# acids-ircam/RAVE

Hardware: NVIDIA H100
Metric: audio-seconds/s (v2 train step fwd+bwd, 48 kHz) (higher is better)
Workload: dtype bf16

## Files before the change

include/rave_b200.h:

```cpp
#ifndef RAVE_B200_H
#define RAVE_B200_H

#include <stddef.h>
#include <stdint.h>

#ifdef __cplusplus
extern "C" {
#endif

#define RAVE_ACT_NONE 0
#define RAVE_ACT_LEAKY 1
#define RAVE_ACT_SNAKE 2

#define RAVE_PREC_FP32 0
#define RAVE_PREC_BF16 1
#define RAVE_PREC_TF32 2

int rave_b200_version(void);
const char *rave_b200_last_error(void);
unsigned long long rave_b200_launch_count(void);

int rave_pqmf_analysis_fwd(const float *x, const float *taps, float *y, int B, int T, int Lout,
                           int ntaps, int pad_l, int flip_sign, void *stream);
int rave_pqmf_synthesis_fwd(const float *x, const float *w, float *out, int B, int L, int K,
// ... 19 lines not shown
                          int Lq, int K, int stride, int dil, int pad_l, long os_a, long os_c,
                          int act_p, int act_q, float slope, const float *alpha, void *workspace,
                          void *stream);

int rave_weight_norm_fwd(const float *v, const float *g, float *w, float *norm_out, int C0, int R,
                         void *stream);
int rave_weight_norm_bwd(const float *dw, const float *v, const float *g, const float *norm,
                         float *dv, float *dg, int C0, int R, void *stream);

int rave_act_fwd(const float *x, float *y, int B, int C, int L, int act, float slope,
                 const float *alpha, void *stream);
int rave_act_bwd(const float *dy, const float *x, float *dx, float *dalpha, int B, int C, int L,
                 int act, float slope, const float *alpha, void *stream);
int rave_am_tanh_fwd(const float *x, float *y, int B, int C, int L, void *stream);
int rave_am_tanh_bwd(const float *dy, const float *x, float *dx, int B, int C, int L, void *stream);
int rave_reparam_fwd(const float *z, const float *eps, float *zs, float *kl_sum, int B, int C, int L, void *stream);

int rave_conv1d_tc_supported(int Cin, int Cout, int K, int stride, int dil);
int rave_dilated_unit_tc_supported(int C, int L);
int rave_dilated_unit_tc_fwd(const void *xa_bf16, const void *w3t_bf16, const void *w1t_bf16, void *a1_out,
                             float *out_f32, void *out_act, int B, int C, int L, int pitch, int dil, int pad_l,
                             float slope_in, float slope_mid, int act_out, float slope_out, void *stream);
int rave_conv1d_tc_plan(int B, int Cin, int Cout, int Lout, int K);
int rave_conv1d_tc_fwd(const void *xa_bf16, const void *wt_bf16, const float *bias, const float *res,
                       const void *res_bf16, const void *dact_src_bf16, const void *res_act_bf16, float res_slope,
                       float *out_f32, void *out_act_bf16,
                       int B, int Cin, int Lin, int in_pitch, int Cout, int Lout,
                       int K, int stride, int dil, int pad_l, int act, float slope, int out_rows,
                       int out_row_stride, int out_row_offset, const float *fm_d, int fm_bh, void *stream);
int rave_conv1d_tc_fwd_x3(const void *xa_bf16, const void *wt_bf16, const float *bias, const float *res,
                          const void *res_act, float res_slope, float *out_f32, void *out_act, int B, int Cin, int Lin,
                          int in_pitch, int Cout, int Lout, int K, int stride, int dil, int pad_l, int act, float slope,
                          int out_rows, int out_row_stride, int out_row_offset, int act_cs, void *stream);
int rave_conv1d_tc_wgrad_splits(int B, int Cm, int Lp, int Cn, int K);
int rave_time_stack_cl(const float *x, void *out_bf16, int B, int C, int T, int F, int Fp, int Cp, int kt, int pt,
                       void *stream);
int rave_time_stack_cl_bwd(const void *g_bf16, float *gx, int B, int C, int T, int F, int Fp, int Cp, int kt, int pt,
                           void *stream);
int rave_time_stack_nhwc(const float *x, void *out_bf16, int B, int C, int T, int F, long sb, long st, int Fp, int Cp, int kt,
                         int pt, void *stream);
int rave_time_stack_nhwc_bwd(const void *g_bf16, float *gx, int B, int C, int T, int F, int Fp, int Cp, int kt, int pt,
                             void *stream);
int rave_time_stack_nhwc_dil(const float *x, void *out_bf16, int B, int C, int T, int F, long sb, long st, int Fp, int Cp,
                             int kt, int pt, int dil, void *stream);
int rave_time_stack_nhwc_dil_bwd(const void *g_bf16, float *gx, int B, int C, int T, int F, int Fp, int Cp, int kt, int pt,
                                 int dil, void *stream);
// ... 109 lines not shown
```

rave_b200/_lib.py:

```python
import ctypes
import os
from ctypes import c_float, c_int, c_long, c_size_t, c_ulonglong, c_void_p, c_char_p

_HERE = os.path.dirname(os.path.abspath(__file__))
LIB_PATH = os.path.join(_HERE, "csrc", "librave_b200.so")

_P, _I, _F, _L = c_void_p, c_int, c_float, c_long

SIGNATURES = {
    "rave_b200_version": (c_int, []),
    "rave_b200_last_error": (c_char_p, []),
    "rave_b200_launch_count": (c_ulonglong, []),
    "rave_pqmf_analysis_fwd": (c_int, [_P, _P, _P, _I, _I, _I, _I, _I, _I, _P]),
    "rave_pqmf_synthesis_fwd": (c_int, [_P, _P, _P, _I, _I, _I, _I, _F, _I, _P]),
    "rave_pqmf_analysis_fast": (c_int, [_P, _P, _P, _P, _I, _I, _I, _I, _I, _P]),
    "rave_pqmf_synthesis_fast": (c_int, [_P, _P, _P, _P, _I, _I, _I, _F, _I, _P]),
    "rave_conv1d_gather_f32": (c_int, [_P, _P, _P, _P, _P, _I, _I, _I, _I, _I, _I, _I, _I, _I, _L, _L,
                                       _I, _F, _P, _I, _F, _P, _P, _P]),
    "rave_conv1d_scatter_f32": (c_int, [_P, _P, _P, _P, _P, _I, _I, _I, _I, _I, _I, _I, _I, _I, _L, _L,
                                        _I, _F, _P, _I, _F, _P, _P, _P]),
    "rave_conv1d_wgrad_workspace_bytes": (c_size_t, [_I, _I, _I, _I, _I]),
    "rave_conv1d_wgrad_f32": (c_int, [_P, _P, _P, _I, _I, _I, _I, _I, _I, _I, _I, _I, _L, _L, _I, _I,
                                      _F, _P, _P, _P]),
    "rave_weight_norm_fwd": (c_int, [_P, _P, _P, _P, _I, _I, _P]),
    "rave_weight_norm_bwd": (c_int, [_P, _P, _P, _P, _P, _P, _I, _I, _P]),
    "rave_act_fwd": (c_int, [_P, _P, _I, _I, _I, _I, _F, _P, _P]),
    "rave_act_bwd": (c_int, [_P, _P, _P, _P, _I, _I, _I, _I, _F, _P, _P]),
    "rave_am_tanh_fwd": (c_int, [_P, _P, _I, _I, _I, _P]),
    "rave_am_tanh_bwd": (c_int, [_P, _P, _P, _I, _I, _I, _P]),
    "rave_reparam_fwd": (c_int, [_P, _P, _P, _P, _I, _I, _I, _P]),
    "rave_conv1d_tc_supported": (c_int, [_I, _I, _I, _I, _I]),
    "rave_dilated_unit_tc_supported": (c_int, [_I, _I]),
    "rave_dilated_unit_tc_fwd": (c_int, [_P, _P, _P, _P, _P, _P, _I, _I, _I, _I, _I, _I, _F, _F, _I, _F, _P]),
    "rave_conv1d_tc_plan": (c_int, [_I, _I, _I, _I, _I]),
    "rave_conv1d_tc_fwd": (c_int, [_P, _P, _P, _P, _P, _P, _P, _F, _P, _P, _I, _I, _I, _I, _I, _I, _I, _I, _I, _I, _I,
                                   _F, _I, _I, _I, _P, _I, _P]),
    "rave_conv1d_tc_fwd_x3": (c_int, [_P, _P, _P, _P, _P, _F, _P, _P, _I, _I, _I, _I, _I, _I, _I, _I, _I, _I, _I, _F, _I,
                                      _I, _I, _I, _P]),
    "rave_weight_prep_tc_multi_x3": (c_int, [_I, _P, _P]),
    "rave_ncl_to_cl_x3": (c_int, [_P, _P, _I, _I, _I, _P]),
    "rave_conv1d_tc_wgrad": (c_int, [_P, _P, _P, _P, _I, _I, _I, _I, _I, _I, _I, _I, _I, _I, _I, _P]),
    "rave_tapmajor_to_weight_f32": (c_int, [_P, _P, _I, _I, _I, _I, _I, _P]),
    "rave_conv1d_tc_wgrad_splits": (c_int, [_I, _I, _I, _I, _I]),
    "rave_time_stack_cl": (c_int, [_P, _P, _I, _I, _I, _I, _I, _I, _I, _I, _P]),
    "rave_time_stack_cl_bwd": (c_int, [_P, _P, _I, _I, _I, _I, _I, _I, _I, _I, _P]),
    "rave_time_stack_nhwc": (c_int, [_P, _P, _I, _I, _I, _I, ctypes.c_long, ctypes.c_long, _I, _I, _I, _I, _P]),
    "rave_time_stack_nhwc_bwd": (c_int, [_P, _P, _I, _I, _I, _I, _I, _I, _I, _I, _P]),
    "rave_time_stack_nhwc_dil": (c_int, [_P, _P, _I, _I, _I, _I, ctypes.c_long, ctypes.c_long, _I, _I, _I, _I, _I, _P]),
    "rave_time_stack_nhwc_dil_bwd": (c_int, [_P, _P, _I, _I, _I, _I, _I, _I, _I, _I, _I, _P]),
    "rave_l1_stats_f32": (c_int, [_P, _P, _P, ctypes.c_long, _P]),
    "rave_leaky_fm_fwd": (c_int, [_P, _P, _P, ctypes.c_long, ctypes.c_float, _P]),
    "rave_leaky_fm_bwd": (c_int, [_P, _P, _P, _P, ctypes.c_long, ctypes.c_float, _P]),
    "rave_leaky_fm_stack_fwd": (c_int, [_P, _P, _P, _P, ctypes.c_long, _I, _I, _I, _I, ctypes.c_float, _P]),
    "rave_leaky_fm_stack_bwd": (c_int, [_P, _P, _P, _P, _P, ctypes.c_long, _I, _I, _I, _I, ctypes.c_float, _P]),
    "rave_leaky_fm_stack_dil_fwd": (c_int, [_P, _P, _P, _P, ctypes.c_long, _I, _I, _I, _I, _I, ctypes.c_float, _P]),
    "rave_leaky_fm_stack_dil_bwd": (c_int, [_P, _P, _P, _P, _P, ctypes.c_long, _I, _I, _I, _I, _I, ctypes.c_float, _P]),
    "rave_l1_grad_f32": (c_int, [_P, _P, _P, _P, _P, ctypes.c_long, _P]),
# ... 119 lines not shown
```

rave_b200/csrc/api.cu:

```cuda
#include <stdarg.h>

#include <atomic>

#include "common.cuh"

namespace rave {
static thread_local char g_err[512] = "";
static std::atomic<unsigned long long> g_launches{0};

void set_error(const char *fmt, ...) {
  va_list ap;
  va_start(ap, fmt);
  vsnprintf(g_err, sizeof(g_err), fmt, ap);
  va_end(ap);
}
void count_launch(int n) { g_launches.fetch_add((unsigned long long)n, std::memory_order_relaxed); }
}

extern "C" int rave_b200_version(void) { return 105; }
extern "C" const char *rave_b200_last_error(void) { return rave::g_err; }
extern "C" unsigned long long rave_b200_launch_count(void) {
  return rave::g_launches.load(std::memory_order_relaxed);
}
```

rave_b200/csrc/conv_tc.cu:

```cuda
#include <string.h>

#include "common.cuh"
#include "tc_common.cuh"

namespace rave {
namespace tc {

constexpr int BLOCK_M = 128;
constexpr int NUM_THREADS = 288;
constexpr int SMEM_MAX = 227 * 1024;

struct TcParams {
  int B, Cin, Lin, Cout, Lout, K, stride, dil, pad_l;
  int BL, BB;
  int n_lt, n_bg, n_nt;
  int num_kb;
  int act;
  float slope;
  const float *bias;
  const float *res;
  const __nv_bfloat16 *res_bf16;
  const __nv_bfloat16 *dact_src;
  const __nv_bfloat16 *res_act;
  float res_inv_slope;
  float *out_f32;
  __nv_bfloat16 *out_act;
  int out_rows;
  int out_row_stride;
  int out_row_offset;
  const float *fm_d;
  long fm_half;
  int fm_bh;
  int x3;
  int act_ld;
  int act_cs;
  int stages, nacc;
  int stg;
  int acc_off, stg_off, bar_off;
};

template <int BLOCK_N, int BLOCK_K, bool X3 = false>
struct SmemLayout {
  static constexpr int PARTS = X3 ? 2 : 1;
  static constexpr int A_PART = BLOCK_M * BLOCK_K * 2;
  static constexpr int B_PART = (BLOCK_N * BLOCK_K * 2 + 1023) / 1024 * 1024;
  static constexpr int A_BYTES = PARTS * A_PART;
  static constexpr int B_BYTES = PARTS * BLOCK_N * BLOCK_K * 2;
  static constexpr int B_BYTES_PAD = PARTS * B_PART;
  static constexpr int STAGE_BYTES = A_BYTES + B_BYTES_PAD;
  static constexpr int ACC_LD = acc_pitch(BLOCK_N);
  static constexpr int ACC_BYTES = BLOCK_M * ACC_LD * 4;
  static constexpr int OUT_BOXC = BLOCK_N % 64 == 0 ? 64 : BLOCK_N % 32 == 0 ? 32 : 16;
  static constexpr int OUT_SPAN = OUT_BOXC * 2;
  static constexpr int STG_BYTES = X3 ? 0 : BLOCK_M * BLOCK_N * 2;
  static constexpr int FIXED = 256 + 1024;
  static constexpr int stages_for(int nacc, int stg) {
    const int s = (SMEM_MAX - FIXED - nacc * ACC_BYTES - stg * STG_BYTES) / STAGE_BYTES;
    return s > 8 ? 8 : s;
  }
};

template <int BLOCK_N, int BLOCK_K, bool X3>
static void plan_smem(int kblocks, TcParams &p) {
  using L = SmemLayout<BLOCK_N, BLOCK_K, X3>;
  const int base = L::stages_for(1, 0);
  const int need = kblocks + 1 < base ? kblocks + 1 : base;
  p.nacc = 1;
  p.stg = 0;
  if (L::stages_for(2, 1) >= need) { p.nacc = 2; p.stg = 1; }
  else if (L::stages_for(1, 1) >= need) p.stg = 1;
  if (X3) p.stg = 0;
  p.stages = L::stages_for(p.nacc, p.stg);
  p.acc_off = p.stages * L::STAGE_BYTES;
  p.stg_off = p.acc_off + p.nacc * L::ACC_BYTES;
  p.bar_off = p.stg_off + p.stg * L::STG_BYTES;
}

template <int BOXC>
__device__ __forceinline__ uint32_t stg_offset(int row, int c) {
  constexpr int SPAN = BOXC * 2;
  const uint32_t line = (uint32_t)row * SPAN;
  const uint32_t piece = (uint32_t)((c % BOXC) >> 3) ^ ((line >> 7) & (SPAN / 16 - 1));
  return (uint32_t)(c / BOXC) * (BLOCK_M * SPAN) + line + (piece << 4);
}

template <int NWORDS>
__device__ __forceinline__ void ld_words(const void *ptr, uint32_t *w) {
  static_assert(NWORDS % 8 == 0, "256-bit granules");
#pragma unroll
  for (int i = 0; i < NWORDS / 8; ++i) ldg256(reinterpret_cast<const uint8_t *>(ptr) + 32 * i, w + 8 * i);
}
template <int NWORDS>
__device__ __forceinline__ void st_words(void *ptr, const uint32_t *w) {
  static_assert(NWORDS % 8 == 0, "256-bit granules");
#pragma unroll
  for (int i = 0; i < NWORDS / 8; ++i) stg256(reinterpret_cast<uint8_t *>(ptr) + 32 * i, w + 8 * i);
}
__device__ __forceinline__ float bf_lo(uint32_t w) { return __uint_as_float(w << 16); }
__device__ __forceinline__ float bf_hi(uint32_t w) { return __uint_as_float(w & 0xFFFF0000u); }

template <int CW, bool X3, int BOXC>
__device__ __forceinline__ void tc_epi_chunk(const TcParams &p, uint32_t taddr, int co, bool valid, size_t orow,
                                             int fm_side, uint8_t *stg, int row, int cl) {
  constexpr int NW = CW / 2;
  float v[CW];
  uint32_t rf[CW], rb[NW], dm[NW], ra[NW], ra2[X3 ? NW : 1], pm[NW];
  const size_t off = orow * p.Cout + co;
  const int cs = X3 ? p.act_cs : 0;
  const size_t offa = X3 ? orow * (size_t)p.act_ld + (size_t)(co / cs) * (2 * cs) + (co % cs) : off;
  if (valid) {
    if (!X3 && fm_side)
      ld_words<NW>(p.dact_src + (fm_side > 0 ? off + p.fm_half : off - p.fm_half), pm);
    if (p.res_act) {
      ld_words<NW>(p.res_act + offa, ra);
      if (X3) ld_words<NW>(p.res_act + offa + cs, ra2);
    }
    if (p.res) ld_words<CW>(p.res + off, rf);
    if (!X3 && p.res_bf16) ld_words<NW>(p.res_bf16 + off, rb);
    if (!X3 && p.dact_src) ld_words<NW>(p.dact_src + off, dm);
  }
  acc_ld<CW>(taddr, v);
  if (!valid) return;
  if (p.bias) {
    const float4 *b4 = reinterpret_cast<const float4 *>(p.bias + co);
#pragma unroll
    for (int i = 0; i < CW / 4; ++i) {
      const float4 bb = __ldg(b4 + i);
      v[4 * i] += bb.x; v[4 * i + 1] += bb.y; v[4 * i + 2] += bb.z; v[4 * i + 3] += bb.w;
    }
  }
  if (!X3 && p.dact_src) {
#pragma unroll
    for (int w = 0; w < NW; ++w) {
      if (dm[w] & 0x00008000u) v[2 * w] *= p.slope;
      if (dm[w] & 0x80000000u) v[2 * w + 1] *= p.slope;
    }
  }
  if (!X3 && fm_side) {
    const float d0 = __ldg(p.fm_d), d1 = fm_side > 0 ? __ldg(p.fm_d + 1) : 0.f;
#pragma unroll
    for (int w = 0; w < NW; ++w) {
#pragma unroll
      for (int h = 0; h < 2; ++h) {
        const float as = h ? bf_hi(dm[w]) : bf_lo(dm[w]);
        const float ap = h ? bf_hi(pm[w]) : bf_lo(pm[w]);
        const float t = (as > ap ? 1.f : 0.f) - (as < ap ? 1.f : 0.f);
        const float sr = (as > 0.f ? 1.f : 0.f) - (as < 0.f ? 1.f : 0.f);
        v[2 * w + h] = fmaf(d1, sr, fmaf(d0, t, v[2 * w + h]));
      }
    }
  }
  if (!X3 && p.res_bf16) {
#pragma unroll
    for (int w = 0; w < NW; ++w) {
      v[2 * w] += bf_lo(rb[w]);
      v[2 * w + 1] += bf_hi(rb[w]);
    }
  }
  if (p.res_act) {
#pragma unroll
    for (int w = 0; w < NW; ++w) {
      float a0 = bf_lo(ra[w]), a1 = bf_hi(ra[w]);
      if (X3) {
        a0 += bf_lo(ra2[w]);
        a1 += bf_hi(ra2[w]);
      }
      v[2 * w] += fminf(a0, a0 * p.res_inv_slope);
      v[2 * w + 1] += fminf(a1, a1 * p.res_inv_slope);
    }
  }
  if (p.res) {
#pragma unroll
    for (int i = 0; i < CW; ++i) v[i] += __uint_as_float(rf[i]);
  }
  if (p.out_f32) {
    uint32_t o[CW];
#pragma unroll
    for (int i = 0; i < CW; ++i) o[i] = __float_as_uint(v[i]);
    st_words<CW>(p.out_f32 + off, o);
  }
  if (p.out_act) {
    uint32_t pk[NW], pl[X3 ? NW : 1];
#pragma unroll
    for (int w = 0; w < NW; ++w) {
      float a0 = v[2 * w], a1 = v[2 * w + 1];
      if (p.act == RAVE_ACT_LEAKY) {
        a0 = fmaxf(a0, a0 * p.slope);
        a1 = fmaxf(a1, a1 * p.slope);
      }
      __nv_bfloat162 h = __floats2bfloat162_rn(a0, a1);
      pk[w] = *reinterpret_cast<uint32_t *>(&h);
      if (X3) {
        __nv_bfloat162 l = __floats2bfloat162_rn(a0 - bf_lo(pk[w]), a1 - bf_hi(pk[w]));
        pl[w] = *reinterpret_cast<uint32_t *>(&l);
      }
    }
    if (!X3 && stg) {
#pragma unroll
      for (int j = 0; j < NW / 4; ++j) sts128(stg + stg_offset<BOXC>(row, cl + 8 * j), pk + 4 * j);
    } else {
      st_words<NW>(p.out_act + offa, pk);
      if (X3) st_words<NW>(p.out_act + offa + cs, pl);
    }
  }
}

template <int BLOCK_N, bool X3, int BOXC>
__device__ __forceinline__ void tc_epilogue(const TcParams &p, uint32_t taddr, int n0, bool valid, size_t orow,
                                            int fm_side, uint8_t *stg, int row) {
  constexpr int MAIN = BLOCK_N / 32 * 32;
  if (X3 && (p.act_cs & 31)) {
#pragma unroll 1
    for (int c0 = 0; c0 < BLOCK_N; c0 += 16)
      tc_epi_chunk<16, X3, BOXC>(p, taddr + c0, n0 + c0, valid, orow, fm_side, stg, row, c0);
    return;
  }
#pragma unroll 1
  for (int c0 = 0; c0 < MAIN; c0 += 32)
    tc_epi_chunk<32, X3, BOXC>(p, taddr + c0, n0 + c0, valid, orow, fm_side, stg, row, c0);
  if (MAIN < BLOCK_N) tc_epi_chunk<16, X3, BOXC>(p, taddr + MAIN, n0 + MAIN, valid, orow, fm_side, stg, row, MAIN);
}

template <int BLOCK_N, int BLOCK_K, bool X3>
__global__ void __launch_bounds__(NUM_THREADS, 1)
conv_tc_kernel(const __grid_constant__ CUtensorMap tmap_a, const __grid_constant__ CUtensorMap tmap_b,
               const __grid_constant__ CUtensorMap tmap_o, const TcParams p) {
  using L = SmemLayout<BLOCK_N, BLOCK_K, X3>;
  const int STAGES = p.stages;
  constexpr int SWZ = BLOCK_K * 2;
  static_assert(BLOCK_N % 16 == 0 && BLOCK_N >= 16 && BLOCK_N <= 128, "invalid wgmma N");

  extern __shared__ uint8_t smem_raw[];
  uint8_t *smem = reinterpret_cast<uint8_t *>((reinterpret_cast<uintptr_t>(smem_raw) + 1023) & ~uintptr_t(1023));
  uint64_t *full_bar = reinterpret_cast<uint64_t *>(smem + p.bar_off);
  uint64_t *empty_bar = full_bar + STAGES;
  uint64_t *tfull_bar = empty_bar + STAGES;
  uint64_t *tempty_bar = tfull_bar + 2;
  uint8_t *stg = (!X3 && p.stg) ? smem + p.stg_off : nullptr;

  const int warp = threadIdx.x >> 5;
  const int lane = threadIdx.x & 31;
  const int num_tiles = p.n_lt * p.n_bg * p.n_nt;
  const int kblocks = p.K * p.num_kb;

  if (threadIdx.x == 0) {
    tma_prefetch_desc(&tmap_a);
    tma_prefetch_desc(&tmap_b);
    if (stg) tma_prefetch_desc(&tmap_o);
    for (int s = 0; s < STAGES; ++s) {
      mbar_init(&full_bar[s], 1);
      mbar_init(&empty_bar[s], 4);
    }
    for (int b = 0; b < 2; ++b) {
      mbar_init(&tfull_bar[b], 128);
      mbar_init(&tempty_bar[b], 4);
    }
    fence_barrier_init();
    acc_bind(smem + p.acc_off, L::ACC_LD);
  }
  __syncthreads();
  griddep_launch_dependents();
  griddep_wait();

  if (warp == 4) {
    int stage = 0;
    uint32_t phase = 0;
    for (int tile = blockIdx.x; tile < num_tiles; tile += gridDim.x) {
      const int nt = tile % p.n_nt;
      const int mt = tile / p.n_nt;
      const int lt = mt % p.n_lt;
      const int bg = mt / p.n_lt;
      const int l0 = lt * p.BL;
      const int b0 = bg * p.BB;
      const int n0 = nt * BLOCK_N;
      for (int k = 0; k < p.K; ++k) {
        const int off = k * p.dil - p.pad_l;
        int j = off / p.stride;
        int ph = off - j * p.stride;
        if (ph < 0) { ph += p.stride; j -= 1; }
// ... 53 lines not shown
        if (kb > 0) {
          __syncwarp();
          if (lane == 0) mbar_arrive(&empty_bar[prev]);
        }
        prev = stage;
        if (++stage == STAGES) { stage = 0; phase ^= 1; }
      }
      wgmma_wait<0>();
      wgmma_fence_regs<BLOCK_N / 2>(d[0]);
      wgmma_fence_regs<BLOCK_N / 2>(d[1]);
      __syncwarp();
      if (lane == 0) mbar_arrive(&empty_bar[prev]);
      const int buf = p.nacc == 2 ? (it & 1) : 0;
      const uint32_t use = p.nacc == 2 ? (it >> 1) : it;
      mbar_wait(&tempty_bar[buf], (use & 1) ^ 1);
      acc_store<BLOCK_N>(d, threadIdx.x, 0, 128 * buf);
      mbar_arrive(&tfull_bar[buf]);
    }
  } else {
    constexpr int BOXC = L::OUT_BOXC;
    const int quad = warp & 3;
    const int row = quad * 32 + lane;
    const bool issuer = threadIdx.x == 160;
    int it = 0;
    for (int tile = blockIdx.x; tile < num_tiles; tile += gridDim.x, ++it) {
      const int nt = tile % p.n_nt;
      const int mt = tile / p.n_nt;
      const int lt = mt % p.n_lt;
      const int bg = mt / p.n_lt;
      const int n0 = nt * BLOCK_N;
      const int b = bg * p.BB + row / p.BL;
      const int l = lt * p.BL + row % p.BL;
      const bool valid = (b < p.B) && (l < p.Lout);
      const size_t orow = (size_t)b * p.out_rows + (size_t)l * p.out_row_stride + p.out_row_offset;

      const int buf = p.nacc == 2 ? (it & 1) : 0;
      const uint32_t use = p.nacc == 2 ? (it >> 1) : it;
      if (stg) {
        if (issuer) bulk_wait_read<0>();
        named_bar_sync(1, 128);
      }
      mbar_wait(&tfull_bar[buf], use & 1);
      const uint32_t taddr = (uint32_t)(128 * buf + quad * 32) << 16;
      tc_epilogue<BLOCK_N, X3, BOXC>(p, taddr, n0, valid, orow, p.fm_d ? (b < p.fm_bh ? 1 : -1) : 0, stg, row);
      __syncwarp();
      if (lane == 0) mbar_arrive(&tempty_bar[buf]);
// ... 35 lines not shown
}

static int pick_block_k(int Cin) {
  if (Cin % 64 == 0) return 64;
  if (Cin % 32 == 0) return 32;
  if (Cin % 16 == 0) return 16;
  return 0;
}

static int pick_block_n(int Cout, long m_tiles) {
  const int cands[] = {128, 96, 64, 48, 32, 16};
  constexpr int NC = sizeof(cands) / sizeof(cands[0]);
  int best = 0;
  for (int c : cands) {
    if (Cout % c) continue;
    if (!best) best = c;
    if (m_tiles * (Cout / c) >= 132) return c;
  }
  for (int i = NC - 1; i >= 0; --i)
    if (Cout % cands[i] == 0 && cands[i] >= 32) return cands[i];
  return best;
}

template <int BN, int BK, bool X3>
static int launch(const CUtensorMap &ta, const CUtensorMap &tb, TcParams p, cudaStream_t stream) {
  using L = SmemLayout<BN, BK, X3>;
  plan_smem<BN, BK, X3>(p.K * p.num_kb, p);
  if (!p.out_act) p.stg = 0;
  const int smem = p.bar_off + L::FIXED;
  static int attr = 0;
  if (smem > attr) {
    cudaError_t e = cudaFuncSetAttribute(conv_tc_kernel<BN, BK, X3>, cudaFuncAttributeMaxDynamicSharedMemorySize, smem);
    if (e != cudaSuccess) {
      set_error("conv1d_tc: cudaFuncSetAttribute(%d bytes): %s", smem, cudaGetErrorString(e));
      return 2;
    }
    attr = smem;
  }
  CUtensorMap to;
  memset(&to, 0, sizeof(to));
  if (p.stg) {
    EncodeTiledFn enc = get_encode_fn();
    cuuint64_t dims[3] = {(cuuint64_t)p.Cout, (cuuint64_t)p.Lout, (cuuint64_t)p.B};
    cuuint64_t strides[2] = {(cuuint64_t)p.Cout * 2 * p.out_row_stride, (cuuint64_t)p.Cout * 2 * p.out_rows};
    cuuint32_t box[3] = {(cuuint32_t)L::OUT_BOXC, (cuuint32_t)p.BL, (cuuint32_t)p.BB};
    cuuint32_t estr[3] = {1, 1, 1};
    CUresult r = enc(&to, CU_TENSOR_MAP_DATA_TYPE_BFLOAT16, 3, p.out_act + (size_t)p.out_row_offset * p.Cout, dims,
                     strides, box, estr, CU_TENSOR_MAP_INTERLEAVE_NONE, swizzle_enum(L::OUT_SPAN),
                     CU_TENSOR_MAP_L2_PROMOTION_NONE, CU_TENSOR_MAP_FLOAT_OOB_FILL_NONE);
    if (r != CUDA_SUCCESS) {
      set_error("conv1d_tc: output tensor map encode failed (%d)", (int)r);
      return 1;
    }
  }
  const int tiles = p.n_lt * p.n_bg * p.n_nt;
  int dev = 0, sms = 132;
  cudaGetDevice(&dev);
  cudaDeviceGetAttribute(&sms, cudaDevAttrMultiProcessorCount, dev);
  const int grid = tiles < sms ? tiles : sms;
  launch_pdl(conv_tc_kernel<BN, BK, X3>, dim3(grid), dim3(NUM_THREADS), smem, stream, ta, tb, to, p);
  RAVE_CHECK_LAUNCH("conv1d_tc");
  return 0;
}

template <int BK, bool X3>
static int dispatch_n(int bn, const CUtensorMap &ta, const CUtensorMap &tb, const TcParams &p,
                      cudaStream_t s) {
  switch (bn) {
    case 128: return launch<128, BK, X3>(ta, tb, p, s);
    case 96: return launch<96, BK, X3>(ta, tb, p, s);
    case 64: return launch<64, BK, X3>(ta, tb, p, s);
    case 48: return launch<48, BK, X3>(ta, tb, p, s);
    case 32: return launch<32, BK, X3>(ta, tb, p, s);
    case 16: return launch<16, BK, X3>(ta, tb, p, s);
  }
  set_error("conv1d_tc: no kernel for BLOCK_N=%d", bn);
  return 1;
}

template <int BK>
static int smem_plan_bits(int BN, int kblocks) {
  TcParams q;
  switch (BN) {
    case 128: plan_smem<128, BK, false>(kblocks, q); break;
    case 96: plan_smem<96, BK, false>(kblocks, q); break;
    case 64: plan_smem<64, BK, false>(kblocks, q); break;
    case 48: plan_smem<48, BK, false>(kblocks, q); break;
    case 32: plan_smem<32, BK, false>(kblocks, q); break;
    case 16: plan_smem<16, BK, false>(kblocks, q); break;
    default: return 0;
  }
  return (q.nacc - 1) << 24 | q.stg << 25 | q.stages << 26;
}

template <bool X3>
static int dispatch_all(int BK, int BN, const CUtensorMap &ta, const CUtensorMap &tb, const TcParams &p, cudaStream_t s) {
  switch (BK) {
    case 64: return dispatch_n<64, X3>(BN, ta, tb, p, s);
    case 32: return dispatch_n<32, X3>(BN, ta, tb, p, s);
    case 16: return dispatch_n<16, X3>(BN, ta, tb, p, s);
  }
  set_error("conv1d_tc: no kernel for BLOCK_K=%d", BK);
  return 1;
}

int conv_tc_dispatch_x3(int BK, int BN, const CUtensorMap &ta, const CUtensorMap &tb, const TcParams &p, cudaStream_t s);
#ifdef RAVE_TC_X3_UNIT
int conv_tc_dispatch_x3(int BK, int BN, const CUtensorMap &ta, const CUtensorMap &tb, const TcParams &p, cudaStream_t s) {
  return dispatch_all<true>(BK, BN, ta, tb, p, s);
}
#endif

}
}

#ifndef RAVE_TC_X3_UNIT
extern "C" int rave_conv1d_tc_supported(int Cin, int Cout, int K, int stride, int dil) {
  if (rave::tc::pick_block_k(Cin) == 0) return 0;
  if (Cout % 16) return 0;
  if (K < 1 || stride < 1 || dil < 1) return 0;
  return 1;
}

extern "C" int rave_conv1d_tc_plan(int B, int Cin, int Cout, int Lout, int K) {
  using namespace rave;
  using namespace rave::tc;
  const int BK = pick_block_k(Cin);
  if (!BK || Cout % 16) return 0;
  int BL = 128;
  while (BL > Lout && BL > 8) BL >>= 1;
  const long m_tiles = (long)ceil_div(Lout, BL) * ceil_div(B, 128 / BL);
  const int BN = pick_block_n(Cout, m_tiles);
  if (!BN) return 0;
  const int kblocks = K * ceil_div(Cin, BK);
  const int smem = BK == 64 ? smem_plan_bits<64>(BN, kblocks)
                 : BK == 32 ? smem_plan_bits<32>(BN, kblocks) : smem_plan_bits<16>(BN, kblocks);
  return BN | (BK << 12) | smem;
}

static int conv1d_tc_fwd_impl(const void *xa, const void *wt, const float *bias, const float *res,
                              const void *res_bf16, const void *dact_src, const void *res_act, float res_slope,
                              float *out_f32, void *out_act,
                              int B, int Cin, int Lin, int in_pitch, int Cout, int Lout,
                              int K, int stride, int dil, int pad_l, int act, float slope, int out_rows,
                              int out_row_stride, int out_row_offset, const float *fm_d, int fm_bh,
                              void *stream, int x3, int act_cs = 0) {
  using namespace rave;
  using namespace rave::tc;
  RAVE_CHECK_ARG(!x3 || (!res_bf16 && !dact_src && !fm_d),
                 "conv1d_tc(x3): the split-operand mode has no gradient epilogues (forward path only)");
  RAVE_CHECK_ARG(xa && wt && (out_f32 || out_act), "conv1d_tc: null pointer");
  RAVE_CHECK_ARG(rave_conv1d_tc_supported(Cin, Cout, K, stride, dil), "conv1d_tc: unsupported shape Cin=%d Cout=%d",
                 Cin, Cout);
  if (in_pitch <= 0) in_pitch = Lin;
  RAVE_CHECK_ARG(in_pitch >= ceil_div(Lin, stride) * stride,
                 "conv1d_tc: input pitch %d < Lin %d rounded up to the stride %d (slack rows must be zero)", in_pitch,
                 Lin, stride);
  RAVE_CHECK_ARG(act == RAVE_ACT_NONE || act == RAVE_ACT_LEAKY, "conv1d_tc: epilogue activation %d unsupported", act);
  RAVE_CHECK_ARG(act != RAVE_ACT_LEAKY || (slope >= 0.f && slope <= 1.f), "conv1d_tc: LeakyReLU slope %g outside [0, 1]",
                 (double)slope);
// ... 21 lines not shown
  p.out_row_offset = out_row_offset;
  RAVE_CHECK_ARG(!fm_d || (dact_src && slope > 0.f && ((fm_bh > 0 && 2 * fm_bh == B) || (fm_bh < 0 && -fm_bh == B))),
                 "conv1d_tc: the fused feature-matching gradient needs dact_src and a [real; fake] batch (B=%d, fm_bh=%d)",
                 B, fm_bh);
  p.fm_d = fm_d;
  p.fm_bh = fm_bh > 0 ? fm_bh : 0;
  p.fm_half = (long)(fm_bh > 0 ? fm_bh : -fm_bh) * p.out_rows * Cout;
  p.x3 = x3 ? 1 : 0;
  p.act_ld = x3 ? 2 * Cout : Cout;
  p.act_cs = act_cs > 0 ? act_cs : Cout;
  RAVE_CHECK_ARG(!x3 || (Cout % p.act_cs == 0 && p.act_cs % 16 == 0),
                 "conv1d_tc(x3): %d channels per position do not tile the %d-column rows in 16-column chunks", p.act_cs,
                 Cout);
  RAVE_CHECK_ARG(!x3 || !res_act || p.act_cs == Cout, "conv1d_tc(x3): res_act needs one position per row");
  int BL = 128;
  while (BL > Lout && BL > 8) BL >>= 1;
  p.BL = BL; p.BB = 128 / BL;
  p.n_lt = ceil_div(Lout, BL);
  p.n_bg = ceil_div(B, p.BB);
  const int BN = pick_block_n(Cout, (long)p.n_lt * p.n_bg);
  RAVE_CHECK_ARG(BN > 0, "conv1d_tc: no BLOCK_N for Cout=%d", Cout);
  p.n_nt = Cout / BN;
  p.num_kb = ceil_div(Cin, BK);

  CUtensorMap ta, tb;
  {
    const cuuint64_t ca = (cuuint64_t)Cin * (x3 ? 2 : 1);
    cuuint64_t dims[4] = {ca, (cuuint64_t)stride, (cuuint64_t)ceil_div(Lin, stride), (cuuint64_t)B};
    cuuint64_t strides[3] = {ca * 2, ca * 2 * stride, ca * 2 * in_pitch};
    cuuint32_t box[4] = {(cuuint32_t)BK, 1, (cuuint32_t)p.BL, (cuuint32_t)p.BB};
    cuuint32_t estr[4] = {1, 1, 1, 1};
    CUresult r = enc(&ta, CU_TENSOR_MAP_DATA_TYPE_BFLOAT16, 4, const_cast<void *>(xa), dims, strides, box, estr,
                     CU_TENSOR_MAP_INTERLEAVE_NONE, swizzle_enum(BK * 2), promo,
                     CU_TENSOR_MAP_FLOAT_OOB_FILL_NONE);
    RAVE_CHECK_ARG(r == CUDA_SUCCESS, "conv1d_tc: tensor map A encode failed (%d)", (int)r);
  }
  {
    cuuint64_t dims[2] = {(cuuint64_t)Cin, (cuuint64_t)K * Cout * (x3 ? 2 : 1)};
    cuuint64_t strides[1] = {(cuuint64_t)Cin * 2};
    cuuint32_t box[2] = {(cuuint32_t)BK, (cuuint32_t)BN};
    cuuint32_t estr[2] = {1, 1};
    CUresult r = enc(&tb, CU_TENSOR_MAP_DATA_TYPE_BFLOAT16, 2, const_cast<void *>(wt), dims, strides, box, estr,
                     CU_TENSOR_MAP_INTERLEAVE_NONE, swizzle_enum(BK * 2), promo,
                     CU_TENSOR_MAP_FLOAT_OOB_FILL_NONE);
    RAVE_CHECK_ARG(r == CUDA_SUCCESS, "conv1d_tc: tensor map B encode failed (%d)", (int)r);
  }
// ... 355 lines not shown
```

Measured before the change: 2013.

## Stage conv epilogue operands through a TMA-fed shared-memory ring with in-place store

Adds a ring-buffer epilogue path to the tensor-core conv kernel. When the gradient-activation source and bf16 output are both present, the dact, feature-matching partner, bf16 residual and activated residual tiles are prefetched by TMA into shared-memory slots. The epilogue reads them from shared memory, writes its result back into the dact slot and stores it with a TMA bulk store, replacing per-thread scattered global loads and stores. The shared memory given to the ring reduces the main-loop pipeline stages and the accumulator buffers, and a new plan query reports the chosen layout.

```diff
diff --git a/include/rave_b200.h b/include/rave_b200.h
--- a/include/rave_b200.h
+++ b/include/rave_b200.h
@@ -65,6 +65,12 @@
                              float *out_f32, void *out_act, int B, int C, int L, int pitch, int dil, int pad_l,
                              float slope_in, float slope_mid, int act_out, float slope_out, void *stream);
 int rave_conv1d_tc_plan(int B, int Cin, int Cout, int Lout, int K);
+#define RAVE_EPI_DACT 1
+#define RAVE_EPI_FM 2
+#define RAVE_EPI_FM_FAKE 4
+#define RAVE_EPI_RES_BF16 8
+#define RAVE_EPI_RES_ACT 16
+int rave_conv1d_tc_plan_epi(int B, int Cin, int Cout, int Lout, int K, int operands);
 int rave_conv1d_tc_fwd(const void *xa_bf16, const void *wt_bf16, const float *bias, const float *res,
                        const void *res_bf16, const void *dact_src_bf16, const void *res_act_bf16, float res_slope,
                        float *out_f32, void *out_act_bf16,
diff --git a/rave_b200/_lib.py b/rave_b200/_lib.py
--- a/rave_b200/_lib.py
+++ b/rave_b200/_lib.py
@@ -33,6 +33,7 @@
     "rave_dilated_unit_tc_supported": (c_int, [_I, _I]),
     "rave_dilated_unit_tc_fwd": (c_int, [_P, _P, _P, _P, _P, _P, _I, _I, _I, _I, _I, _I, _F, _F, _I, _F, _P]),
     "rave_conv1d_tc_plan": (c_int, [_I, _I, _I, _I, _I]),
+    "rave_conv1d_tc_plan_epi": (c_int, [_I, _I, _I, _I, _I, _I]),
     "rave_conv1d_tc_fwd": (c_int, [_P, _P, _P, _P, _P, _P, _P, _F, _P, _P, _I, _I, _I, _I, _I, _I, _I, _I, _I, _I, _I,
                                    _F, _I, _I, _I, _P, _I, _P]),
     "rave_conv1d_tc_fwd_x3": (c_int, [_P, _P, _P, _P, _P, _F, _P, _P, _I, _I, _I, _I, _I, _I, _I, _I, _I, _I, _I, _F, _I,
diff --git a/rave_b200/csrc/api.cu b/rave_b200/csrc/api.cu
--- a/rave_b200/csrc/api.cu
+++ b/rave_b200/csrc/api.cu
@@ -17,7 +17,7 @@
 void count_launch(int n) { g_launches.fetch_add((unsigned long long)n, std::memory_order_relaxed); }
 }
 
-extern "C" int rave_b200_version(void) { return 105; }
+extern "C" int rave_b200_version(void) { return 106; }
 extern "C" const char *rave_b200_last_error(void) { return rave::g_err; }
 extern "C" unsigned long long rave_b200_launch_count(void) {
   return rave::g_launches.load(std::memory_order_relaxed);
diff --git a/rave_b200/csrc/conv_tc.cu b/rave_b200/csrc/conv_tc.cu
--- a/rave_b200/csrc/conv_tc.cu
+++ b/rave_b200/csrc/conv_tc.cu
@@ -37,6 +37,10 @@
   int stages, nacc;
   int stg;
   int acc_off, stg_off, bar_off;
+  int ring, ring_off;
+  int box_d, box_p, box_r, box_a;
+  int nbox, npb;
+  int inplace;
 };
 
 template <int BLOCK_N, int BLOCK_K, bool X3 = false>
@@ -53,27 +57,49 @@
   static constexpr int OUT_BOXC = BLOCK_N % 64 == 0 ? 64 : BLOCK_N % 32 == 0 ? 32 : 16;
   static constexpr int OUT_SPAN = OUT_BOXC * 2;
   static constexpr int STG_BYTES = X3 ? 0 : BLOCK_M * BLOCK_N * 2;
+  static constexpr int RCW = BLOCK_N % 32 == 0 ? 32 : 16;
+  static constexpr int BOX_BYTES = BLOCK_M * RCW * 2;
   static constexpr int FIXED = 256 + 1024;
-  static constexpr int stages_for(int nacc, int stg) {
-    const int s = (SMEM_MAX - FIXED - nacc * ACC_BYTES - stg * STG_BYTES) / STAGE_BYTES;
+  static constexpr int stages_for(int nacc, int stg, int ring_bytes = 0) {
+    const int s = (SMEM_MAX - FIXED - nacc * ACC_BYTES - stg * STG_BYTES - ring_bytes) / STAGE_BYTES;
     return s > 8 ? 8 : s;
   }
 };
 
+constexpr int RING_MAX_KBLOCKS = 24;
+
 template <int BLOCK_N, int BLOCK_K, bool X3>
-static void plan_smem(int kblocks, TcParams &p) {
+static void plan_smem(int kblocks, TcParams &p, int nbox = 0, bool inplace = false) {
   using L = SmemLayout<BLOCK_N, BLOCK_K, X3>;
   const int base = L::stages_for(1, 0);
   const int need = kblocks + 1 < base ? kblocks + 1 : base;
   p.nacc = 1;
   p.stg = 0;
-  if (L::stages_for(2, 1) >= need) { p.nacc = 2; p.stg = 1; }
-  else if (L::stages_for(1, 1) >= need) p.stg = 1;
-  if (X3) p.stg = 0;
-  p.stages = L::stages_for(p.nacc, p.stg);
+  p.ring = 0;
+  p.inplace = 0;
+  if (!X3 && nbox > 0 && inplace && kblocks < RING_MAX_KBLOCKS) {
+    const int floor = need < 3 ? need : 3;
+    const int slot = nbox * L::BOX_BYTES;
+    const int cand[3][2] = {{2, 4}, {1, 4}, {1, 3}};
+    for (int i = 0; i < 3; ++i)
+      if (L::stages_for(cand[i][0], 0, cand[i][1] * slot) >= floor) {
+        p.nacc = cand[i][0];
+        p.ring = cand[i][1];
+        p.inplace = 1;
+        break;
+      }
+  }
+  if (!p.ring) {
+    if (L::stages_for(2, 1) >= need) { p.nacc = 2; p.stg = 1; }
+    else if (L::stages_for(1, 1) >= need) p.stg = 1;
+    if (X3) p.stg = 0;
+  }
+  const int ring_bytes = p.ring * nbox * L::BOX_BYTES;
+  p.stages = L::stages_for(p.nacc, p.stg, ring_bytes);
   p.acc_off = p.stages * L::STAGE_BYTES;
   p.stg_off = p.acc_off + p.nacc * L::ACC_BYTES;
-  p.bar_off = p.stg_off + p.stg * L::STG_BYTES;
+  p.ring_off = p.stg_off + p.stg * L::STG_BYTES;
+  p.bar_off = p.ring_off + ring_bytes;
 }
 
 template <int BOXC>
@@ -99,28 +125,40 @@
 __device__ __forceinline__ float bf_lo(uint32_t w) { return __uint_as_float(w << 16); }
 __device__ __forceinline__ float bf_hi(uint32_t w) { return __uint_as_float(w & 0xFFFF0000u); }
 
-template <int CW, bool X3, int BOXC>
+template <int CW>
+__device__ __forceinline__ void lds_row(const uint8_t *box, int row, uint32_t *w) {
+#pragma unroll
+  for (int j = 0; j < CW / 8; ++j) lds128(box + stg_offset<CW>(row, 8 * j), w + 4 * j);
+}
+
+template <int CW, bool X3, int BOXC, bool RING = false>
 __device__ __forceinline__ void tc_epi_chunk(const TcParams &p, uint32_t taddr, int co, bool valid, size_t orow,
-                                             int fm_side, uint8_t *stg, int row, int cl) {
+                                             int fm_side, uint8_t *stg, int row, int cl, uint8_t *slot, int pbox) {
   constexpr int NW = CW / 2;
+  constexpr int BOX = BLOCK_M * CW * 2;
   float v[CW];
   uint32_t rf[CW], rb[NW], dm[NW], ra[NW], ra2[X3 ? NW : 1], pm[NW];
   const size_t off = orow * p.Cout + co;
   const int cs = X3 ? p.act_cs : 0;
   const size_t offa = X3 ? orow * (size_t)p.act_ld + (size_t)(co / cs) * (2 * cs) + (co % cs) : off;
   if (valid) {
-    if (!X3 && fm_side)
-      ld_words<NW>(p.dact_src + (fm_side > 0 ? off + p.fm_half : off - p.fm_half), pm);
-    if (p.res_act) {
-      ld_words<NW>(p.res_act + offa, ra);
-      if (X3) ld_words<NW>(p.res_act + offa + cs, ra2);
+    if (!RING) {
+      if (!X3 && fm_side)
+        ld_words<NW>(p.dact_src + (fm_side > 0 ? off + p.fm_half : off - p.fm_half), pm);
+      if (p.res_act) {
+        ld_words<NW>(p.res_act + offa, ra);
+        if (X3) ld_words<NW>(p.res_act + offa + cs, ra2);
+      }
     }
     if (p.res) ld_words<CW>(p.res + off, rf);
-    if (!X3 && p.res_bf16) ld_words<NW>(p.res_bf16 + off, rb);
-    if (!X3 && p.dact_src) ld_words<NW>(p.dact_src + off, dm);
+    if (!RING) {
+      if (!X3 && p.res_bf16) ld_words<NW>(p.res_bf16 + off, rb);
+      if (!X3 && p.dact_src) ld_words<NW>(p.dact_src + off, dm);
+    }
   }
   acc_ld<CW>(taddr, v);
   if (!valid) return;
+  if (!X3 && RING && p.dact_src) lds_row<CW>(slot + p.box_d * BOX, row, dm);
   if (p.bias) {
     const float4 *b4 = reinterpret_cast<const float4 *>(p.bias + co);
 #pragma unroll
@@ -138,6 +176,7 @@
   }
   if (!X3 && fm_side) {
     const float d0 = __ldg(p.fm_d), d1 = fm_side > 0 ? __ldg(p.fm_d + 1) : 0.f;
+    if (RING) lds_row<CW>(slot + pbox * BOX, row, pm);
 #pragma unroll
     for (int w = 0; w < NW; ++w) {
 #pragma unroll
@@ -151,6 +190,7 @@
     }
   }
   if (!X3 && p.res_bf16) {
+    if (RING) lds_row<CW>(slot + p.box_r * BOX, row, rb);
 #pragma unroll
     for (int w = 0; w < NW; ++w) {
       v[2 * w] += bf_lo(rb[w]);
@@ -158,6 +198,7 @@
     }
   }
   if (p.res_act) {
+    if (!X3 && RING) lds_row<CW>(slot + p.box_a * BOX, row, ra);
 #pragma unroll
     for (int w = 0; w < NW; ++w) {
       float a0 = bf_lo(ra[w]), a1 = bf_hi(ra[w]);
@@ -195,7 +236,10 @@
         pl[w] = *reinterpret_cast<uint32_t *>(&l);
       }
     }
-    if (!X3 && stg) {
+    if (!X3 && RING) {
+#pragma unroll
+      for (int j = 0; j < NW / 4; ++j) sts128(slot + p.box_d * BOX + stg_offset<CW>(row, 8 * j), pk + 4 * j);
+    } else if (!X3 && stg) {
 #pragma unroll
       for (int j = 0; j < NW / 4; ++j) sts128(stg + stg_offset<BOXC>(row, cl + 8 * j), pk + 4 * j);
     } else {
@@ -212,19 +256,53 @@
   if (X3 && (p.act_cs & 31)) {
 #pragma unroll 1
     for (int c0 = 0; c0 < BLOCK_N; c0 += 16)
-      tc_epi_chunk<16, X3, BOXC>(p, taddr + c0, n0 + c0, valid, orow, fm_side, stg, row, c0);
+      tc_epi_chunk<16, X3, BOXC>(p, taddr + c0, n0 + c0, valid, orow, fm_side, stg, row, c0, nullptr, 0);
     return;
   }
 #pragma unroll 1
   for (int c0 = 0; c0 < MAIN; c0 += 32)
-    tc_epi_chunk<32, X3, BOXC>(p, taddr + c0, n0 + c0, valid, orow, fm_side, stg, row, c0);
-  if (MAIN < BLOCK_N) tc_epi_chunk<16, X3, BOXC>(p, taddr + MAIN, n0 + MAIN, valid, orow, fm_side, stg, row, MAIN);
+    tc_epi_chunk<32, X3, BOXC>(p, taddr + c0, n0 + c0, valid, orow, fm_side, stg, row, c0, nullptr, 0);
+  if (MAIN < BLOCK_N)
+    tc_epi_chunk<16, X3, BOXC>(p, taddr + MAIN, n0 + MAIN, valid, orow, fm_side, stg, row, MAIN, nullptr, 0);
+}
+
+template <int BLOCK_N, int RCW>
+__device__ __forceinline__ void ring_load(const TcParams &p, const CUtensorMap *md, const CUtensorMap *mp,
+                                          const CUtensorMap *mr, const CUtensorMap *ma, uint8_t *ring,
+                                          uint64_t *rfull, int num_tiles, int g) {
+  constexpr int NCH = BLOCK_N / RCW, BOX = BLOCK_M * RCW * 2;
+  const int tile = blockIdx.x + (g / NCH) * gridDim.x;
+  if (tile >= num_tiles) return;
+  const int nt = tile % p.n_nt;
+  const int mt = tile / p.n_nt;
+  const int lt = mt % p.n_lt;
+  const int bg = mt / p.n_lt;
+  const int c0 = nt * BLOCK_N + (g % NCH) * RCW, l0 = lt * p.BL, b0 = bg * p.BB;
+  const int slot = g % p.ring;
+  uint8_t *sp = ring + slot * (p.nbox * BOX);
+  uint64_t *bar = rfull + slot;
+  bool p0 = false, p1 = false;
+  int s0 = 0;
+  if (p.box_p >= 0) {
+    if (p.fm_bh == 0) p0 = true;
+    else if (p.npb == 1) { p0 = true; s0 = b0 < p.fm_bh ? p.fm_bh : -p.fm_bh; }
+    else { p0 = b0 < p.fm_bh; p1 = b0 + p.BB > p.fm_bh; s0 = p.fm_bh; }
+  }
+  const int skipped = p.npb == 2 ? (int)!p0 + (int)!p1 : 0;
+  mbar_arrive_expect_tx(bar, (uint32_t)((p.nbox - skipped) * BOX));
+  if (p.box_d >= 0) tma_load_3d(sp + p.box_d * BOX, md, bar, c0, l0, b0);
+  if (p0) tma_load_3d(sp + p.box_p * BOX, mp, bar, c0, l0, b0 + s0);
+  if (p1) tma_load_3d(sp + (p.box_p + 1) * BOX, mp, bar, c0, l0, b0 - p.fm_bh);
+  if (p.box_r >= 0) tma_load_3d(sp + p.box_r * BOX, mr, bar, c0, l0, b0);
+  if (p.box_a >= 0) tma_load_3d(sp + p.box_a * BOX, ma, bar, c0, l0, b0);
 }
 
 template <int BLOCK_N, int BLOCK_K, bool X3>
 __global__ void __launch_bounds__(NUM_THREADS, 1)
 conv_tc_kernel(const __grid_constant__ CUtensorMap tmap_a, const __grid_constant__ CUtensorMap tmap_b,
-               const __grid_constant__ CUtensorMap tmap_o, const TcParams p) {
+               const __grid_constant__ CUtensorMap tmap_o, const __grid_constant__ CUtensorMap tmap_d,
+               const __grid_constant__ CUtensorMap tmap_p, const __grid_constant__ CUtensorMap tmap_r,
+               const __grid_constant__ CUtensorMap tmap_ra, const TcParams p) {
   using L = SmemLayout<BLOCK_N, BLOCK_K, X3>;
   const int STAGES = p.stages;
   constexpr int SWZ = BLOCK_K * 2;
@@ -236,7 +314,9 @@
   uint64_t *empty_bar = full_bar + STAGES;
   uint64_t *tfull_bar = empty_bar + STAGES;
   uint64_t *tempty_bar = tfull_bar + 2;
+  uint64_t *rfull_bar = tempty_bar + 2;
   uint8_t *stg = (!X3 && p.stg) ? smem + p.stg_off : nullptr;
+  const int ring = X3 ? 0 : p.ring;
 
   const int warp = threadIdx.x >> 5;
   const int lane = threadIdx.x & 31;
@@ -246,7 +326,13 @@
   if (threadIdx.x == 0) {
     tma_prefetch_desc(&tmap_a);
     tma_prefetch_desc(&tmap_b);
-    if (stg) tma_prefetch_desc(&tmap_o);
+    if (stg || p.inplace) tma_prefetch_desc(&tmap_o);
+    if (ring) {
+      if (p.box_d >= 0) tma_prefetch_desc(&tmap_d);
+      if (p.box_p >= 0) tma_prefetch_desc(&tmap_p);
+      if (p.box_r >= 0) tma_prefetch_desc(&tmap_r);
+      if (p.box_a >= 0) tma_prefetch_desc(&tmap_ra);
+    }
     for (int s = 0; s < STAGES; ++s) {
       mbar_init(&full_bar[s], 1);
       mbar_init(&empty_bar[s], 4);
@@ -255,6 +341,7 @@
       mbar_init(&tfull_bar[b], 128);
       mbar_init(&tempty_bar[b], 4);
     }
+    for (int s = 0; s < ring; ++s) mbar_init(&rfull_bar[s], 1);
     fence_barrier_init();
     acc_bind(smem + p.acc_off, L::ACC_LD);
   }
@@ -354,6 +441,55 @@
     const int quad = warp & 3;
     const int row = quad * 32 + lane;
     const bool issuer = threadIdx.x == 160;
+    constexpr int RCW = L::RCW, NCH = BLOCK_N / RCW, RBOX = L::BOX_BYTES;
+    if (ring) {
+      uint8_t *ring_base = smem + p.ring_off;
+      if (issuer)
+        for (int g = 0; g < ring; ++g)
+          ring_load<BLOCK_N, RCW>(p, &tmap_d, &tmap_p, &tmap_r, &tmap_ra, ring_base, rfull_bar, num_tiles, g);
+      int it = 0;
+      for (int tile = blockIdx.x; tile < num_tiles; tile += gridDim.x, ++it) {
+        const int nt = tile % p.n_nt;
+        const int mt = tile / p.n_nt;
+        const int lt = mt % p.n_lt;
+        const int bg = mt / p.n_lt;
+        const int n0 = nt * BLOCK_N;
+        const int b = bg * p.BB + row / p.BL;
+        const int l = lt * p.BL + row % p.BL;
+        const bool valid = (b < p.B) && (l < p.Lout);
+        const size_t orow = (size_t)b * p.out_rows + (size_t)l * p.out_row_stride + p.out_row_offset;
+        const int fm_side = p.fm_d ? (b < p.fm_bh ? 1 : -1) : 0;
+        const int pbox = p.box_p + ((p.npb == 2 && fm_side < 0) ? 1 : 0);
+        const int buf = p.nacc == 2 ? (it & 1) : 0;
+        const uint32_t use = p.nacc == 2 ? (it >> 1) : it;
+        mbar_wait(&tfull_bar[buf], use & 1);
+        const uint32_t taddr = (uint32_t)(128 * buf + quad * 32) << 16;
+#pragma unroll 1
+        for (int c = 0; c < NCH; ++c) {
+          const int g = it * NCH + c;
+          const int slot = g % p.ring;
+          uint8_t *sp = ring_base + slot * (p.nbox * RBOX);
+          mbar_wait(&rfull_bar[slot], (uint32_t)(g / p.ring) & 1);
+          tc_epi_chunk<RCW, X3, BOXC, true>(p, taddr + c * RCW, n0 + c * RCW, valid, orow, fm_side, nullptr, row,
+                                            c * RCW, sp, pbox);
+          fence_proxy_async();
+          named_bar_sync(1, 128);
+          if (issuer) {
+            tma_store_3d(&tmap_o, sp + p.box_d * RBOX, n0 + c * RCW, lt * p.BL, bg * p.BB);
+            bulk_commit();
+            if (g > 0) {
+              bulk_wait_read<1>();
+              ring_load<BLOCK_N, RCW>(p, &tmap_d, &tmap_p, &tmap_r, &tmap_ra, ring_base, rfull_bar, num_tiles,
+                                      g - 1 + p.ring);
+            }
+          }
+        }
+        __syncwarp();
+        if (lane == 0) mbar_arrive(&tempty_bar[buf]);
+      }
+      if (issuer) bulk_wait_all();
+      return;
+    }
     int it = 0;
     for (int tile = blockIdx.x; tile < num_tiles; tile += gridDim.x, ++it) {
       const int nt = tile % p.n_nt;
@@ -435,11 +571,40 @@
   return best;
 }
 
+static CUresult encode_rows(CUtensorMap *m, const void *base, const TcParams &p, int boxc, CUtensorMapL2promotion promo) {
+  EncodeTiledFn enc = get_encode_fn();
+  cuuint64_t dims[3] = {(cuuint64_t)p.Cout, (cuuint64_t)p.Lout, (cuuint64_t)p.B};
+  cuuint64_t strides[2] = {(cuuint64_t)p.Cout * 2 * p.out_row_stride, (cuuint64_t)p.Cout * 2 * p.out_rows};
+  cuuint32_t box[3] = {(cuuint32_t)boxc, (cuuint32_t)p.BL, (cuuint32_t)p.BB};
+  cuuint32_t estr[3] = {1, 1, 1};
+  return enc(m, CU_TENSOR_MAP_DATA_TYPE_BFLOAT16, 3,
+             const_cast<uint8_t *>(reinterpret_cast<const uint8_t *>(base)) + (size_t)p.out_row_offset * p.Cout * 2,
+             dims, strides, box, estr, CU_TENSOR_MAP_INTERLEAVE_NONE, swizzle_enum(boxc * 2), promo,
+             CU_TENSOR_MAP_FLOAT_OOB_FILL_NONE);
+}
+
+static void plan_boxes(TcParams &p, bool dact, bool fm, int fm_bh, bool res_bf16, bool res_act, bool x3) {
+  int n = 0;
+  p.box_d = p.box_p = p.box_r = p.box_a = -1;
+  p.npb = fm && fm_bh > 0 && p.BB > 1 ? 2 : 1;
+  if (!x3) {
+    if (dact) p.box_d = n++;
+    if (fm) { p.box_p = n; n += p.npb; }
+    if (res_bf16) p.box_r = n++;
+    if (res_act) p.box_a = n++;
+  }
+  p.nbox = n;
+}
+
 template <int BN, int BK, bool X3>
 static int launch(const CUtensorMap &ta, const CUtensorMap &tb, TcParams p, cudaStream_t stream) {
   using L = SmemLayout<BN, BK, X3>;
-  plan_smem<BN, BK, X3>(p.K * p.num_kb, p);
+  plan_smem<BN, BK, X3>(p.K * p.num_kb, p, p.nbox, p.dact_src != nullptr && p.out_act != nullptr);
   if (!p.out_act) p.stg = 0;
+  if (p.stages < 2) {
+    set_error("conv1d_tc: shared-memory plan leaves %d main-loop stages (BLOCK_N=%d, BLOCK_K=%d)", p.stages, BN, BK);
+    return 1;
+  }
   const int smem = p.bar_off + L::FIXED;
   static int attr = 0;
   if (smem > attr) {
@@ -450,19 +615,28 @@
     }
     attr = smem;
   }
-  CUtensorMap to;
+  CUtensorMap to, td, tp, tr, tra;
   memset(&to, 0, sizeof(to));
-  if (p.stg) {
-    EncodeTiledFn enc = get_encode_fn();
-    cuuint64_t dims[3] = {(cuuint64_t)p.Cout, (cuuint64_t)p.Lout, (cuuint64_t)p.B};
-    cuuint64_t strides[2] = {(cuuint64_t)p.Cout * 2 * p.out_row_stride, (cuuint64_t)p.Cout * 2 * p.out_rows};
-    cuuint32_t box[3] = {(cuuint32_t)L::OUT_BOXC, (cuuint32_t)p.BL, (cuuint32_t)p.BB};
-    cuuint32_t estr[3] = {1, 1, 1};
-    CUresult r = enc(&to, CU_TENSOR_MAP_DATA_TYPE_BFLOAT16, 3, p.out_act + (size_t)p.out_row_offset * p.Cout, dims,
-                     strides, box, estr, CU_TENSOR_MAP_INTERLEAVE_NONE, swizzle_enum(L::OUT_SPAN),
-                     CU_TENSOR_MAP_L2_PROMOTION_NONE, CU_TENSOR_MAP_FLOAT_OOB_FILL_NONE);
+  memset(&td, 0, sizeof(td));
+  memset(&tp, 0, sizeof(tp));
+  memset(&tr, 0, sizeof(tr));
+  memset(&tra, 0, sizeof(tra));
+  CUresult r = CUDA_SUCCESS;
+  if (p.inplace) r = encode_rows(&to, p.out_act, p, L::RCW, CU_TENSOR_MAP_L2_PROMOTION_NONE);
+  else if (p.stg) r = encode_rows(&to, p.out_act, p, L::OUT_BOXC, CU_TENSOR_MAP_L2_PROMOTION_NONE);
+  if (r != CUDA_SUCCESS) {
+    set_error("conv1d_tc: output tensor map encode failed (%d)", (int)r);
+    return 1;
+  }
+  if (p.ring) {
+    const CUtensorMapL2promotion op = CU_TENSOR_MAP_L2_PROMOTION_L2_256B;
+    if (p.box_d >= 0 && r == CUDA_SUCCESS) r = encode_rows(&td, p.dact_src, p, L::RCW, op);
+    if (p.box_p >= 0 && r == CUDA_SUCCESS)
+      r = encode_rows(&tp, p.fm_bh == 0 ? p.dact_src - p.fm_half : p.dact_src, p, L::RCW, op);
+    if (p.box_r >= 0 && r == CUDA_SUCCESS) r = encode_rows(&tr, p.res_bf16, p, L::RCW, op);
+    if (p.box_a >= 0 && r == CUDA_SUCCESS) r = encode_rows(&tra, p.res_act, p, L::RCW, op);
     if (r != CUDA_SUCCESS) {
-      set_error("conv1d_tc: output tensor map encode failed (%d)", (int)r);
+      set_error("conv1d_tc: epilogue operand tensor map encode failed (%d)", (int)r);
       return 1;
     }
   }
@@ -471,7 +645,7 @@
   cudaGetDevice(&dev);
   cudaDeviceGetAttribute(&sms, cudaDevAttrMultiProcessorCount, dev);
   const int grid = tiles < sms ? tiles : sms;
-  launch_pdl(conv_tc_kernel<BN, BK, X3>, dim3(grid), dim3(NUM_THREADS), smem, stream, ta, tb, to, p);
+  launch_pdl(conv_tc_kernel<BN, BK, X3>, dim3(grid), dim3(NUM_THREADS), smem, stream, ta, tb, to, td, tp, tr, tra, p);
   RAVE_CHECK_LAUNCH("conv1d_tc");
   return 0;
 }
@@ -492,18 +666,21 @@
 }
 
 template <int BK>
-static int smem_plan_bits(int BN, int kblocks) {
-  TcParams q;
+static bool smem_plan(int BN, int kblocks, TcParams &q, bool inplace) {
   switch (BN) {
-    case 128: plan_smem<128, BK, false>(kblocks, q); break;
-    case 96: plan_smem<96, BK, false>(kblocks, q); break;
-    case 64: plan_smem<64, BK, false>(kblocks, q); break;
-    case 48: plan_smem<48, BK, false>(kblocks, q); break;
-    case 32: plan_smem<32, BK, false>(kblocks, q); break;
-    case 16: plan_smem<16, BK, false>(kblocks, q); break;
-    default: return 0;
-  }
-  return (q.nacc - 1) << 24 | q.stg << 25 | q.stages << 26;
+    case 128: plan_smem<128, BK, false>(kblocks, q, q.nbox, inplace); break;
+    case 96: plan_smem<96, BK, false>(kblocks, q, q.nbox, inplace); break;
+    case 64: plan_smem<64, BK, false>(kblocks, q, q.nbox, inplace); break;
+    case 48: plan_smem<48, BK, false>(kblocks, q, q.nbox, inplace); break;
+    case 32: plan_smem<32, BK, false>(kblocks, q, q.nbox, inplace); break;
+    case 16: plan_smem<16, BK, false>(kblocks, q, q.nbox, inplace); break;
+    default: return false;
+  }
+  return true;
+}
+static bool smem_plan_bk(int BK, int BN, int kblocks, TcParams &q, bool inplace) {
+  return BK == 64 ? smem_plan<64>(BN, kblocks, q, inplace)
+       : BK == 32 ? smem_plan<32>(BN, kblocks, q, inplace) : smem_plan<16>(BN, kblocks, q, inplace);
 }
 
 template <bool X3>
@@ -535,20 +712,37 @@
   return 1;
 }
 
-extern "C" int rave_conv1d_tc_plan(int B, int Cin, int Cout, int Lout, int K) {
+static bool tc_plan(int B, int Cin, int Cout, int Lout, int K, int operands, int *BN, int *BK, rave::tc::TcParams &q) {
   using namespace rave;
   using namespace rave::tc;
-  const int BK = pick_block_k(Cin);
-  if (!BK || Cout % 16) return 0;
+  *BK = pick_block_k(Cin);
+  if (!*BK || Cout % 16) return false;
   int BL = 128;
   while (BL > Lout && BL > 8) BL >>= 1;
-  const long m_tiles = (long)ceil_div(Lout, BL) * ceil_div(B, 128 / BL);
-  const int BN = pick_block_n(Cout, m_tiles);
-  if (!BN) return 0;
-  const int kblocks = K * ceil_div(Cin, BK);
-  const int smem = BK == 64 ? smem_plan_bits<64>(BN, kblocks)
-                 : BK == 32 ? smem_plan_bits<32>(BN, kblocks) : smem_plan_bits<16>(BN, kblocks);
-  return BN | (BK << 12) | smem;
+  q.BL = BL;
+  q.BB = 128 / BL;
+  const long m_tiles = (long)ceil_div(Lout, BL) * ceil_div(B, q.BB);
+  *BN = pick_block_n(Cout, m_tiles);
+  if (!*BN) return false;
+  const bool dact = operands & (RAVE_EPI_DACT | RAVE_EPI_FM | RAVE_EPI_FM_FAKE);
+  const bool fm = operands & (RAVE_EPI_FM | RAVE_EPI_FM_FAKE);
+  plan_boxes(q, dact, fm, (operands & RAVE_EPI_FM) ? B / 2 : -B, operands & RAVE_EPI_RES_BF16,
+             operands & RAVE_EPI_RES_ACT, false);
+  return smem_plan_bk(*BK, *BN, K * ceil_div(Cin, *BK), q, dact);
+}
+
+extern "C" int rave_conv1d_tc_plan(int B, int Cin, int Cout, int Lout, int K) {
+  int BN, BK;
+  rave::tc::TcParams q;
+  if (!tc_plan(B, Cin, Cout, Lout, K, 0, &BN, &BK, q)) return 0;
+  return BN | (BK << 12) | (q.nacc - 1) << 24 | q.stg << 25 | q.stages << 26;
+}
+
+extern "C" int rave_conv1d_tc_plan_epi(int B, int Cin, int Cout, int Lout, int K, int operands) {
+  int BN, BK;
+  rave::tc::TcParams q;
+  if (!tc_plan(B, Cin, Cout, Lout, K, operands, &BN, &BK, q)) return 0;
+  return BN | BK << 8 | q.stages << 16 | (q.nacc - 1) << 20 | q.stg << 21 | q.inplace << 22 | q.ring << 24;
 }
 
 static int conv1d_tc_fwd_impl(const void *xa, const void *wt, const float *bias, const float *res,
@@ -616,6 +810,7 @@
   RAVE_CHECK_ARG(BN > 0, "conv1d_tc: no BLOCK_N for Cout=%d", Cout);
   p.n_nt = Cout / BN;
   p.num_kb = ceil_div(Cin, BK);
+  plan_boxes(p, dact_src != nullptr, fm_d != nullptr, fm_bh, res_bf16 != nullptr, res_act != nullptr, x3 != 0);
 
   CUtensorMap ta, tb;
   {
```

Result: faster. 2071 (median of 6 runs) (+2.9%).
